# SamsungLabs/nb-asr

Hardware: NVIDIA B200
Metric: train_utterances_per_sec (higher is better)
Workload: dtype bf16

## Files before the change

include/nbasr.h:

```cpp
#ifndef NBASR_H
#define NBASR_H

#include <stdint.h>

#ifdef __cplusplus
extern "C" {
#endif

#define NBASR_F32 0
#define NBASR_BF16 1
#define NBASR_F16 2
#define NBASR_PAD_L 8
#define NBASR_PAD_R 4
#define NBASR_MAX_ADD 3

typedef struct nbasr_epilogue {
  const float* bias;
  int32_t relu20;
  float drop_p;
  uint64_t drop_seed;
  const uint64_t* drop_step;
  int32_t n_add;
  const void* add[NBASR_MAX_ADD];
  int32_t add_dtype;
// ... 49 lines not shown
  const void* w;
  int32_t w_packed;
  nbasr_epilogue epi;
} nbasr_gconv;

int nbasr_gconv_fwd(const nbasr_gconv* p, void* stream);
int nbasr_gconv_chain(const nbasr_gconv* nodes, int n, int fused, void* work, int64_t work_bytes, void* stream);
int64_t nbasr_gconv_chain_work_bytes(int B, int T, int C, int cpg, int n);
int nbasr_pack_gconv_dgrad(const float* w, float* wt, int C, int cpg, int ktaps, void* stream);
int nbasr_pack_gconv_mma(const float* w, void* out, int out_dtype, int C, int cpg, int ktaps, int transposed, void* stream);
int64_t nbasr_gconv_mma_pack_elems(int C, int cpg, int ktaps);
int nbasr_gconv_wgrad(int dtype, const void* dz, const void* x, int B, int T, int Tp, int C, int cpg,
                      int ktaps, int off0, int dstep, float* dw, float* dbias, void* stream);
int nbasr_gconv_wgrad_x(int dz_dtype, const void* dz, const void* x, int x_dtype, float x_scale, int B, int T, int Tp, int C,
                        int cpg, int ktaps, int off0, int dstep, float* dw, float* dbias, void* stream);

int nbasr_eltwise(int src_dtype, const void* src, int64_t ld_src, int B, int T, int Tp, int C,
                  const nbasr_epilogue* epi, void* stream);

int nbasr_colsum(int dtype, const void* x, int B, int T, int Tp, int C, float* out, void* stream);

int nbasr_layernorm_fwd(int dtype, const void* x, void* y, int B, int T, int Tp, int C,
                        const float* gamma, const float* beta, float eps, float* mean, float* rstd,
                        float out_scale, void* y2, void* stream);
int nbasr_layernorm_bwd(int dtype, const void* dy, const void* x, int x_dtype, float x_scale, const float* mean,
                        const float* rstd, const float* gamma, int B, int T, int Tp, int C, void* dx, void* dx2,
                        const uint32_t* mask2, float scale2, int64_t mask_rows, int mask2_w, float* dgamma,
                        float* dbeta, void* stream);

int nbasr_transpose_in(const float* audio, void* out, int dtype, int B, int F, int T, int Tp, float scale, void* stream);
// ... 86 lines not shown
```

nb_asr_b200/_lib.py:

```python
import ctypes as C
import os

from . import _build

F32, BF16, F16 = 0, 1, 2
PAD_L, PAD_R = 8, 4
MAX_ADD = 3

_vp, _i32, _i64, _f32, _u64 = C.c_void_p, C.c_int32, C.c_int64, C.c_float, C.c_uint64


class Epilogue(C.Structure):
    _fields_ = [('bias', _vp), ('relu20', _i32), ('drop_p', _f32), ('drop_seed', _u64), ('drop_step', _vp),
                ('n_add', _i32), ('add', _vp * MAX_ADD), ('add_dtype', _i32), ('out', _vp), ('out_dtype', _i32),
                ('ld_out', _i64), ('mask_out', _vp), ('out2', _vp), ('out2_dtype', _i32), ('mask2', _vp),
                ('scale2', _f32), ('mask_rows', _i64), ('mask_w', _i32), ('mask2_w', _i32), ('accumulate', _i32),
                ('acc_scale', _f32), ('bias_scale', _f32), ('relu_hi', _f32)]


class Gemm(C.Structure):
    _fields_ = [('dtype', _i32), ('a', _vp), ('a_bs', _i64), ('a_rs', _i64), ('nb', _i32), ('nr', _i32),
                ('K', _i32), ('N', _i32), ('w', _vp), ('ldw', _i64), ('o_r0', _i64), ('o_bs', _i64),
                ('o_rs', _i64), ('epi', Epilogue)]


class Wgrad(C.Structure):
    _fields_ = [('dtype', _i32), ('dy', _vp), ('dy_bs', _i64), ('dy_rs', _i64), ('x', _vp), ('x_bs', _i64),
                ('x_rs', _i64), ('nb', _i32), ('nr', _i32), ('M', _i32), ('N', _i32), ('dw', _vp), ('ldw', _i64), ('dbias', _vp)]


class PackJob(C.Structure):
    _fields_ = [('kind', _i32), ('out_dtype', _i32), ('src', _vp), ('dst', _vp), ('n_out', _i64), ('a', _i32 * 8), ('s', _i64 * 3)]


class GConv(C.Structure):
    _fields_ = [('dtype', _i32), ('x', _vp), ('B', _i32), ('T', _i32), ('Tp', _i32), ('C', _i32), ('cpg', _i32),
                ('ktaps', _i32), ('off0', _i32), ('dstep', _i32), ('w', _vp), ('w_packed', _i32), ('epi', Epilogue)]


class GateLayer(C.Structure):
    _fields_ = [('mask', _vp), ('mask_rows', _i64), ('w', _i32), ('C', _i32), ('Tp', _i32), ('T', _i32), ('s', _i32),
                ('reserved', _i32)]


_SIGS = {
    'nbasr_gemm_tn': [C.POINTER(Gemm), _vp],
    'nbasr_gemm_wgrad': [C.POINTER(Wgrad), _vp],
    'nbasr_gconv_fwd': [C.POINTER(GConv), _vp],
    'nbasr_gconv_chain': [C.POINTER(GConv), C.c_int, C.c_int, _vp, _i64, _vp],
    'nbasr_gconv_chain_work_bytes': [C.c_int] * 5,
    'nbasr_pack_gconv_dgrad': [_vp, _vp, C.c_int, C.c_int, C.c_int, _vp],
    'nbasr_pack_gconv_mma': [_vp, _vp, C.c_int, C.c_int, C.c_int, C.c_int, C.c_int, _vp],
    'nbasr_gconv_mma_pack_elems': [C.c_int, C.c_int, C.c_int],
    'nbasr_gconv_wgrad': [C.c_int, _vp, _vp] + [C.c_int] * 8 + [_vp, _vp, _vp],
    'nbasr_gconv_wgrad_x': [C.c_int, _vp, _vp, C.c_int, _f32] + [C.c_int] * 8 + [_vp, _vp, _vp],
    'nbasr_eltwise': [C.c_int, _vp, _i64, C.c_int, C.c_int, C.c_int, C.c_int, C.POINTER(Epilogue), _vp],
    'nbasr_colsum': [C.c_int, _vp, C.c_int, C.c_int, C.c_int, C.c_int, _vp, _vp],
    'nbasr_layernorm_fwd': [C.c_int, _vp, _vp, C.c_int, C.c_int, C.c_int, C.c_int, _vp, _vp, _f32, _vp, _vp, _f32, _vp, _vp],
    'nbasr_layernorm_bwd': [C.c_int, _vp, _vp, C.c_int, _f32, _vp, _vp, _vp, C.c_int, C.c_int, C.c_int, C.c_int, _vp, _vp, _vp,
                            _f32, _i64, C.c_int, _vp, _vp, _vp],
    'nbasr_transpose_in': [_vp, _vp, C.c_int, C.c_int, C.c_int, C.c_int, C.c_int, _f32, _vp],
    'nbasr_transpose_out': [_vp, _vp, C.c_int, C.c_int, C.c_int, C.c_int, _vp],
    'nbasr_param_stats': [_vp, _vp, _vp, _vp, C.c_int, _i64, _vp, _vp, _vp],
    'nbasr_row_gram': [_vp, C.c_int, _i64, _i64, _vp, _vp, _vp, _vp],
    'nbasr_gate_gram': [_vp, C.c_int, _vp, C.c_int, _vp, _vp, _vp],
    'nbasr_gate_gram_work_elems': [C.c_int],
    'nbasr_pack_weight': [_vp, _vp, C.c_int, C.c_int, C.c_int, C.c_int, C.c_int, C.c_int, _i64, _i64, _i64, _vp],
    'nbasr_convert': [_vp, _vp, C.c_int, _i64, _vp],
    'nbasr_lstm_fwd': [_vp, _vp, C.c_int, C.c_int, C.c_int, _vp, C.c_int, _i64, _i64, _i64, _vp, _vp, _vp, _vp, _vp],
    'nbasr_lstm_bwd': [_vp, _i64, _i64, _i64, _vp, _vp, _vp, C.c_int, C.c_int, C.c_int, _vp, _vp, _vp, _vp, _vp],
# ... 60 lines not shown
```

nb_asr_b200/csrc/gconv.cu:

```cuda
#include <algorithm>

#include "common.cuh"
#include "kernels.h"

namespace {

constexpr int G_TT = 64;
constexpr int G_FB = 16;
constexpr int G_MAXHALO = 12;
constexpr int G_NT = 256;

__host__ __device__ inline int slab_channels(int cpg) {
  return cpg == 10 ? 160 : 96;
}
__host__ __device__ inline int wpitch(int cpg, int ktaps) {
  int p = cpg * ktaps;
  return (p & 1) ? p : p + 1;
}

template <typename T>
__global__ void __launch_bounds__(G_NT) gconv_fwd_kernel(nbasr_gconv p) {
  extern __shared__ float smem[];
  const int CS = slab_channels(p.cpg);
  const int halo = (p.ktaps - 1) * p.dstep;
// ... 222 lines not shown
  if (packed) return sm100_gconv_chain(nodes, n, fused, work, work_bytes, as_stream(stream));
  for (int i = 0; i < n; ++i)
    if (nbasr_gconv_fwd(nodes + i, stream)) return 1;
  return 0;
}

int64_t nbasr_gconv_chain_work_bytes(int B, int T, int C, int cpg, int n) { return sm100_gconv_chain_work_bytes(B, T, C, cpg, n); }

int nbasr_pack_gconv_dgrad(const float* w, float* wt, int C, int cpg, int ktaps, void* stream) {
  int total = C * cpg * ktaps;
  pack_gconv_dgrad_kernel<<<(total + 255) / 256, 256, 0, as_stream(stream)>>>(w, wt, C, cpg, ktaps);
  NBASR_CHECK_LAUNCH();
  return 0;
}

int nbasr_gconv_wgrad_x(int dz_dtype, const void* dz, const void* x, int x_dtype, float x_scale, int B, int T, int Tp, int C,
                        int cpg, int ktaps, int off0, int dstep, float* dw, float* dbias, void* stream) {
  NBASR_REQUIRE(cpg == 6 || cpg == 8 || cpg == 10 || cpg == 12, "cpg");
  NBASR_REQUIRE(ktaps <= 7 && (dstep == 1 || dstep == 2), "taps");
  NBASR_REQUIRE(dz_dtype == NBASR_BF16 ? (x_dtype == NBASR_BF16 || x_dtype == NBASR_F16) : (dz_dtype == NBASR_F32 && x_dtype == NBASR_F32),
                "dtypes: bf16 dz with bf16 / fp16 x, or fp32 dz and x");
  if (B <= 0 || T <= 0) return 0;
  if (dz_dtype == NBASR_BF16 && !nbasr_env_flag(NBASR_ENV_FORCE_SIMT))
    return sm100_gconv_wgrad(dz, x, x_dtype == NBASR_F16, x_scale, B, T, Tp, C, cpg, ktaps, off0, dstep, dw, dbias, as_stream(stream));
  if (dbias && nbasr_colsum(dz_dtype, dz, B, T, Tp, C, dbias, stream)) return 1;
  int CS = slab_channels(cpg);
  dim3 grid((C + CS - 1) / CS, B);
  size_t sm = wgrad_smem(cpg);
  auto launch = [&](auto kern, auto dzp, auto xp) {
    static DevOnce attr;
    if (!attr) { cudaFuncSetAttribute(kern, cudaFuncAttributeMaxDynamicSharedMemorySize, 200 * 1024); attr = true; }
    kern<<<grid, G_NT, sm, as_stream(stream)>>>(dzp, xp, x_scale, B, T, Tp, C, cpg, ktaps, off0, dstep, dw);
  };
  if (dz_dtype == NBASR_F32) launch(gconv_wgrad_kernel<float, float>, (const float*)dz, (const float*)x);
  else if (x_dtype == NBASR_F16) launch(gconv_wgrad_kernel<bf16, f16>, (const bf16*)dz, (const f16*)x);
  else launch(gconv_wgrad_kernel<bf16, bf16>, (const bf16*)dz, (const bf16*)x);
  NBASR_CHECK_LAUNCH();
  return 0;
}

int nbasr_gconv_wgrad(int dtype, const void* dz, const void* x, int B, int T, int Tp, int C, int cpg, int ktaps,
                      int off0, int dstep, float* dw, float* dbias, void* stream) {
  return nbasr_gconv_wgrad_x(dtype, dz, x, dtype, 1.f, B, T, Tp, C, cpg, ktaps, off0, dstep, dw, dbias, stream);
}

}
```

nb_asr_b200/csrc/gconv_sm100.cu:

```cuda
#include <cuda.h>

#include "common.cuh"
#include "kernels.h"
#include "sm100_ptx.cuh"
#include "gconv_sm100.cuh"

using namespace sm100;

namespace {

struct GcFwdArgs {
  int B, T, C, OUT, ktaps, dstep, off0;
  int nslabs, ntiles, tiles_per_utt, nlanes, nstage, no_prefetch, w_stable, f16;
  nbasr_epilogue epi;
  int64_t Tp;
};


__global__ void __launch_bounds__(FWD_THREADS, 2)
gconv_mma_fwd_kernel(const __grid_constant__ CUtensorMap tmX, const __grid_constant__ CUtensorMap tmW,
                     const __grid_constant__ CUtensorMap tmO, const __grid_constant__ CUtensorMap tmO2, const GcFwdArgs p) {
  extern __shared__ uint8_t smem_raw[];
  const uint32_t base = (smem_u32(smem_raw) + 1023u) & ~1023u;
  uint8_t* al = smem_raw + (base - smem_u32(smem_raw));
// ... 207 lines not shown
      }
    }
    if (hh == 0 && lane == 0) bulk_wait0();
  }
  tcgen05_fence_before();
  __syncthreads();
  if (warp == W_MMA) {
    tcgen05_fence_after();
    tmem_dealloc(tm, 256);
  }
}

constexpr int DZROWS = 136;
constexpr int DZ_BYTES = DZROWS * 128;
constexpr int WG_STAGE = DZ_BYTES + A_BYTES;
constexpr int WG_SMEM = NSTAGE * WG_STAGE + 1024 + 256;

struct GcWgArgs {
  int B, T, C, cpg, OUT, ktaps, dstep, off0;
  int nslabs, nchunks, nunits, nlanes, dbg;
  int x_f16;
  float x_scale;
  float* dw;
  float* dbias;
};

__global__ void __launch_bounds__(GC_THREADS, 2)
gconv_mma_wgrad_kernel(const __grid_constant__ CUtensorMap tmDZ, const __grid_constant__ CUtensorMap tmX, const GcWgArgs p) {
  extern __shared__ uint8_t smem_raw[];
  const uint32_t base = (smem_u32(smem_raw) + 1023u) & ~1023u;
  uint8_t* al = smem_raw + (base - smem_u32(smem_raw));
  const uint32_t bar0 = base + NSTAGE * WG_STAGE;
  auto full_bar = [&](int s) { return bar0 + 8u * s; };
  auto empty_bar = [&](int s) { return bar0 + 8u * (NSTAGE + s); };
  const uint32_t tfull = bar0 + 8u * (2 * NSTAGE);
  auto ready_bar = [&](int s) { return bar0 + 8u * (2 * NSTAGE + 1 + s); };
  uint32_t* tptr = reinterpret_cast<uint32_t*>(al + NSTAGE * WG_STAGE + 8 * (3 * NSTAGE + 2));
  const int warp = uniform_warp_idx(), lane = threadIdx.x & 31;
  const int slab = blockIdx.x % p.nslabs;
  const int lane_id = blockIdx.x / p.nslabs;
  const int c0 = slab * p.OUT;
  const int cbox = c0 & ~7, coff = c0 - cbox;
  const int npairs = (p.ktaps + 1) / 2;

  if (warp == 4 && lane == 0) {
    prefetch_tmap(&tmDZ);
    prefetch_tmap(&tmX);
    for (int s = 0; s < NSTAGE; ++s) { mbar_init(full_bar(s), 1); mbar_init(empty_bar(s), 1); mbar_init(ready_bar(s), 4); }
    mbar_init(tfull, 1);
    fence_barrier_init();
  }
  if (warp == 5) tmem_alloc(smem_u32(tptr), 256);
  pdl_launch_dependents();
  tcgen05_fence_before();
  __syncthreads();
  tcgen05_fence_after();
  const uint32_t tm = *tptr;
  pdl_wait();
  const bool has_work = lane_id < p.nunits;

  if (warp == 4) {
    if (lane == 0) {
      int stage = 0;
      uint32_t phase = 0;
      for (int u = lane_id; u < p.nunits; u += p.nlanes) {
        const int b = u / p.nchunks, t0 = (u % p.nchunks) * GT;
        mbar_wait(empty_bar(stage), phase ^ 1);
        mbar_expect_tx(full_bar(stage), DZ_BYTES + A_BYTES);
        const uint32_t sa = base + stage * WG_STAGE;
        tma_load_3d(sa, &tmDZ, full_bar(stage), cbox, NBASR_PAD_L + t0 - p.dstep, b);
        tma_load_3d(sa + DZ_BYTES, &tmX, full_bar(stage), cbox, NBASR_PAD_L + t0 + p.off0, b);
        if (++stage == NSTAGE) { stage = 0; phase ^= 1; }
      }
    }
  } else if (warp == 5) {
    if (has_work) {
      const uint32_t idesc = make_idesc(128, 64 * npairs, 1, 1);
      int stage = 0;
      uint32_t phase = 0;
      bool first = true;
      for (int u = lane_id; u < p.nunits; u += p.nlanes) {
        mbar_wait((p.x_f16 || p.dbias) ? ready_bar(stage) : full_bar(stage), phase);
        const uint32_t sa = base + stage * WG_STAGE;
        tcgen05_fence_after();
        const uint64_t ad0 = make_smem_desc(sa, (uint32_t)p.dstep * 128u, 1024);
        const uint64_t bd0 = make_smem_desc(sa + DZ_BYTES, 2u * (uint32_t)p.dstep * 128u, 1024);
        if (elect_one()) {
#pragma unroll
          for (int k = 0; k < GT / 16; ++k)
            if (!(p.dbg & 2048) || k == 0) umma_bf16(tm, ad0 + (uint64_t)(k * 128), bd0 + (uint64_t)(k * 128), idesc, (!first || k > 0) ? 1u : 0u);
          umma_commit(empty_bar(stage));
        }
        __syncwarp();
        first = false;
        if (++stage == NSTAGE) { stage = 0; phase ^= 1; }
      }
      if (elect_one()) umma_commit(tfull);
      __syncwarp();
    }
  } else if (has_work) {
    if (p.x_f16 || p.dbias) {
      constexpr int QROWS = AROWS / 4;
      const int r0 = warp * QROWS;
      int stage = 0;
      uint32_t phase = 0;
      for (int u = lane_id; u < p.nunits; u += p.nlanes) {
        mbar_wait(full_bar(stage), phase);
        uint8_t* xb = al + stage * WG_STAGE + DZ_BYTES;
        if (p.x_f16) {
#pragma unroll 3
          for (int i = lane; i < QROWS * 8; i += 32) {
            const int r = r0 + (i >> 3), ch = i & 7;
            uint4* cp = reinterpret_cast<uint4*>(xb + r * 128 + ch * 16);
            uint4 w = *cp;
            uint32_t* h = &w.x;
#pragma unroll
            for (int e = 0; e < 4; ++e) {
              const float2 f = f16x2_to_f2(h[e]);
              h[e] = f2_to_bf16x2(f.x * p.x_scale, f.y * p.x_scale);
            }
            if (p.dbias && ch == (7 ^ (r & 7))) w.w = (w.w & 0xffffu) | (0x3F80u << 16);
            *cp = w;
          }
        } else {
          for (int r = r0 + lane; r < r0 + QROWS; r += 32)
            *reinterpret_cast<uint16_t*>(xb + r * 128 + ((7 ^ (r & 7)) << 4) + 14) = 0x3F80;
        }
        asm volatile("fence.proxy.async.shared::cta;" ::: "memory");
        __syncwarp();
        if (lane == 0) mbar_arrive(ready_bar(stage));
        if (++stage == NSTAGE) { stage = 0; phase ^= 1; }
      }
    }
    const int q = warp & 3;
    const int m = q * 32 + lane;
    const int half = m >> 6, co_l = m & 63;
    const int co = cbox + co_l;
    const bool row_ok = co_l >= coff && co_l < coff + p.OUT && co < p.C;
    const int g_l = (co_l - coff) / p.cpg;
    const int nco = min(p.OUT, p.C - c0);
    const int nrun = nco * p.cpg * p.ktaps;
    float* g = p.dw + (int64_t)c0 * p.cpg * p.ktaps;
    const int head = min(nrun, (int)(((16u - (uint32_t)(reinterpret_cast<uintptr_t>(g) & 15u)) & 15u) >> 2));
    float* run = reinterpret_cast<float*>(al) + ((4 - head) & 3);
    mbar_wait(tfull, 0);
    tcgen05_fence_after();
    for (int pr = 0; pr < npairs; ++pr) {
      float v[64];
      const uint32_t ta = tm + ((uint32_t)(q * 32) << 16) + pr * 64;
      tmem_ld32(ta, v);
      tmem_ld32(ta + 32, v + 32);
      const int tap = half ? 2 * pr : 2 * pr + 1;
      if (pr == 0 && p.dbias && row_ok && half) atomicAdd(p.dbias + co, v[63]);
      if (row_ok && tap < p.ktaps) {
        float* dst = run + (co_l - coff) * p.cpg * p.ktaps + tap;
#pragma unroll
        for (int i = 0; i < 64; ++i) {
          const int il = i - coff - g_l * p.cpg;
          if (il >= 0 && il < p.cpg) dst[il * p.ktaps] = v[i];
        }
      }
    }
    named_bar_sync(1, 128);
    if (!(p.dbg & 1024)) {
      const int tid = threadIdx.x;
      const int nvec = (nrun - head) >> 2, tail = head + 4 * nvec;
      if (tid < head) atomicAdd(g + tid, run[tid]);
      for (int j = tid; j < nvec; j += 128)
        atomicAdd(reinterpret_cast<float4*>(g + head) + j, reinterpret_cast<const float4*>(run + head)[j]);
      if (tail + tid < nrun) atomicAdd(g + tail + tid, run[tail + tid]);
    }
  }
  tcgen05_fence_before();
  __syncthreads();
  if (warp == 5) {
    tcgen05_fence_after();
    tmem_dealloc(tm, 256);
  }
}

template <typename T>
__global__ void pack_gconv_mma_kernel(const float* __restrict__ w, T* __restrict__ out, int C, int cpg, int ktaps, int OUT,
                                      int nslabs, int transposed) {
  int64_t idx = (int64_t)blockIdx.x * blockDim.x + threadIdx.x;
  int64_t total = (int64_t)nslabs * ktaps * NW * 64;
  if (idx >= total) return;
  int kk = (int)(idx % 64);
  int n = (int)((idx / 64) % NW);
  int j = (int)((idx / (64 * NW)) % ktaps);
  int s = (int)(idx / ((int64_t)64 * NW * ktaps));
  int c0 = s * OUT;
  int cn = c0 + n, ck = c0 + kk;
// ... 41 lines not shown
  if (sm100_get_map(o1, 3, dx, sx, bo, &tmO, 0)) return 1;
  if (sm100_get_map(o2, 3, dx, sx, bo, &tmO2, 0)) return 1;
  NBASR_REQUIRE(!g->epi.mask_out || g->epi.mask_w == a.OUT, "grouped-conv mask planes are slab wide");
  size_t smem = (size_t)a.ktaps * WTAP_BYTES + (size_t)a.nstage * A_BYTES + 2 * OSTAGE_BYTES + 1024 + 256 + 1024;
  static DevOnce attr;
  if (!attr) {
    cudaError_t e = cudaFuncSetAttribute(gconv_mma_fwd_kernel, cudaFuncAttributeMaxDynamicSharedMemorySize, FWD_SMEM_BUDGET);
    if (e != cudaSuccess) return nbasr_fail("gconv_mma_fwd smem attr: %s", cudaGetErrorString(e));
    attr = true;
  }
  cudaError_t le = launch_pdl(gconv_mma_fwd_kernel, dim3(a.nslabs * a.nlanes), dim3(FWD_THREADS), smem, st, 1, tmX, tmW, tmO, tmO2, a);
  if (le != cudaSuccess) return nbasr_fail("gconv_mma_fwd launch: %s", cudaGetErrorString(le));
  return 0;
}

int sm100_gconv_wgrad(const void* dz, const void* x, int x_f16, float x_scale, int B, int T, int Tp, int C, int cpg, int ktaps,
                      int off0, int dstep, float* dw, float* dbias, cudaStream_t st) {
  GcWgArgs a{};
  a.x_f16 = x_f16;
  a.x_scale = x_scale;
  a.B = B; a.T = T; a.C = C; a.cpg = cpg; a.OUT = wg_slab_out(cpg); a.ktaps = ktaps; a.dstep = dstep; a.off0 = off0;
  NBASR_REQUIRE(off0 >= -NBASR_PAD_L && (ktaps - 1) * dstep <= AROWS - GT && dstep <= DZROWS - GT, "tap reach");
  a.nslabs = (C + a.OUT - 1) / a.OUT;
  a.nchunks = (T + dstep + GT - 1) / GT;
  a.nunits = a.nchunks * B;
  int slots = GCONV_SLOTS * nbasr_sm_count();
  a.nlanes = std::max(1, std::min(a.nunits, slots / a.nslabs));
  a.dw = dw;
  a.dbias = dbias;
  a.dbg = nbasr_env_chain_dbg();
  CUtensorMap tmDZ, tmX;
  uint64_t dd[3] = {(uint64_t)C, (uint64_t)Tp, (uint64_t)B};
  int64_t sd[3] = {1, C, (int64_t)Tp * C};
  uint32_t bz[3] = {64, DZROWS, 1};
  uint32_t bx[3] = {64, AROWS, 1};
  if (sm100_get_map(dz, 3, dd, sd, bz, &tmDZ)) return 1;
  if (sm100_get_map(x, 3, dd, sd, bx, &tmX)) return 1;
  static DevOnce attr;
  if (!attr) {
    cudaError_t e = cudaFuncSetAttribute(gconv_mma_wgrad_kernel, cudaFuncAttributeMaxDynamicSharedMemorySize, WG_SMEM);
    if (e != cudaSuccess) return nbasr_fail("gconv_mma_wgrad smem attr: %s", cudaGetErrorString(e));
    attr = true;
  }
  cudaError_t le = launch_pdl(gconv_mma_wgrad_kernel, dim3(a.nslabs * a.nlanes), dim3(GC_THREADS), (size_t)WG_SMEM, st, 1, tmDZ, tmX, a);
  if (le != cudaSuccess) return nbasr_fail("gconv_mma_wgrad launch: %s", cudaGetErrorString(le));
  return 0;
}

extern "C" int nbasr_pack_gconv_mma(const float* w, void* out, int out_dtype, int C, int cpg, int ktaps, int transposed, void* stream) {
  int OUT = slab_out(cpg);
  int nslabs = (C + OUT - 1) / OUT;
  int64_t total = (int64_t)nslabs * ktaps * NW * 64;
  NBASR_REQUIRE(out_dtype == NBASR_BF16 || out_dtype == NBASR_F16, "16-bit pack");
  const unsigned grid = (unsigned)((total + 255) / 256);
  if (out_dtype == NBASR_F16) pack_gconv_mma_kernel<f16><<<grid, 256, 0, as_stream(stream)>>>(w, (f16*)out, C, cpg, ktaps, OUT, nslabs, transposed);
  else pack_gconv_mma_kernel<bf16><<<grid, 256, 0, as_stream(stream)>>>(w, (bf16*)out, C, cpg, ktaps, OUT, nslabs, transposed);
  NBASR_CHECK_LAUNCH();
  return 0;
}
// ... 6 lines not shown
```

nb_asr_b200/csrc/gconv_sm100.cuh:

```cuda
#pragma once
#include "sm100_ptx.cuh"

namespace {
using namespace sm100;

constexpr int GT = 128;
constexpr int AROWS = 144;
constexpr int A_BYTES = AROWS * 128;
constexpr int NW = 48;
constexpr int WTAP_BYTES = NW * 128;
constexpr int NSTAGE = 3;
constexpr int NACC = 4;
constexpr int GC_THREADS = 192;
constexpr int FWD_THREADS = 448;
constexpr int NEPI = 384;
constexpr int OSTAGE_BYTES = GT * NW * 2;
constexpr int FWD_SMEM_BUDGET = 112 * 1024;

__host__ __device__ inline int slab_out(int cpg) { return cpg == 10 ? 40 : 48; }
__host__ __device__ inline int wg_slab_out(int cpg) { return (56 / cpg) * cpg; }
__host__ __device__ inline int fwd_nstage(int ktaps) {
  int n = (FWD_SMEM_BUDGET - 3072 - ktaps * WTAP_BYTES - 2 * OSTAGE_BYTES) / A_BYTES;
  return n > 4 ? 4 : n;
}


constexpr int GCONV_SLOTS = 2;
}
// ... 1 lines not shown
```

nb_asr_b200/csrc/kernels.h:

```cpp
#pragma once
#include <cuda_runtime.h>
#include <stdint.h>

#include "../../include/nbasr.h"

enum NbasrEnvFlag { NBASR_ENV_FORCE_SIMT = 0, NBASR_ENV_NO_PDL, NBASR_ENV_GCONV_NO_PREFETCH, NBASR_ENV_LSTM_SS, NBASR_ENV_DEBUG,
                    NBASR_ENV_GEMM_DIRECT_EPI, NBASR_ENV_WGRAD_V1, NBASR_ENV_COUNT };
bool nbasr_env_flag(int which);
int nbasr_env_gemm_bn();
int nbasr_env_gemm_l2pf();
int nbasr_env_chain_dbg();
double nbasr_env_wgrad_epi_us();

struct DevOnce {
  unsigned long long mask = 0;
  static int dev() { int d = 0; cudaGetDevice(&d); return d & 63; }
  bool operator!() const { return !((mask >> dev()) & 1ull); }
  DevOnce& operator=(bool v) { if (v) mask |= 1ull << dev(); return *this; }
};

#ifdef __CUDACC__
#include <utility>
template <typename... KArgs, typename... Args>
inline cudaError_t launch_pdl(void (*kern)(KArgs...), dim3 grid, dim3 block, size_t smem, cudaStream_t st, int cluster_x,
// ... 29 lines not shown
  int64_t o_r0, o_bs, o_rs;
  nbasr_epilogue epi;
};
int simt_gemm_launch(const SimtGemmArgs& a, cudaStream_t st);

int sm100_gemm_tn_pair(const nbasr_gemm* p, cudaStream_t st);
int sm100_gemm_wgrad_pair(const nbasr_wgrad* p, cudaStream_t st);

struct CUtensorMap_st;
int sm100_get_map(const void* base, int rank, const uint64_t* dims, const int64_t* strides_el, const uint32_t* box,
                  CUtensorMap_st* out, int swizzle128 = 1);

int sm100_gconv_fwd(const nbasr_gconv* p, cudaStream_t st);
int sm100_gconv_chain(const nbasr_gconv* nodes, int n, int fused, void* work, int64_t work_bytes, cudaStream_t st);
int64_t sm100_gconv_chain_work_bytes(int B, int T, int C, int cpg, int n);
int sm100_gconv_wgrad(const void* dz, const void* x, int x_f16, float x_scale, int B, int T, int Tp, int C, int cpg, int ktaps,
                      int off0, int dstep, float* dw, float* dbias, cudaStream_t st);

int sm100_lstm_fwd(const float* gx, const void* w_packed, int T, int B, int H, void* h_seq, int h_dtype, int64_t h_bs, int64_t h_rs,
                   float* gates, float* cstate, cudaStream_t st);
int sm100_lstm_bwd(const float* dh_seq, int64_t dh_bs, int64_t dh_rs, const void* w_packed, const float* gates, const float* cstate,
                   int T, int B, int H, float* dgx, void* dgx_bf16, cudaStream_t st);

int ln2_fwd(const void* x, void* y, int f16, int B, int T, int Tp, int C, const float* gamma, const float* beta, float eps, float* mean,
            float* rstd, float out_scale, void* y2, cudaStream_t st);
int ln2_bwd(const void* dy, const void* x, int x_f16, float x_scale, const float* mean, const float* rstd, const float* gamma, int B, int T,
            int Tp, int C, void* dx, void* dx2, const uint32_t* mask2, float scale2, int64_t mask_rows, int mask2_w, float* dgamma,
            float* dbeta, cudaStream_t st);
```

nb_asr_b200/engine.py:

```python
import collections
import ctypes as C
import functools
import math
import os

import torch

from . import _lib
from ._lib import BF16, F16, F32, PAD_L, PAD_R, Epilogue, GConv, Gemm, Wgrad
from .model import CELLS_PER_BLOCK, CONV_EDGES, FEATURES, FILTERS, HIDDEN, TR_STRIDES, PadConvRelu, pad_rule

HP = 512
ACT_SCALE = 32.0


def _ptr(t, off_elems=0):
    return t.data_ptr() + off_elems * t.element_size()


def dense_wgrad_inputs(arch, use_norm, use_rnn, input_dropout=False):
    ops = [nd[0] for nd in arch]
    names = {'input'}
    for i, ncells in enumerate(CELLS_PER_BLOCK):
        cin = f'b{i}.ln'
# ... 734 lines not shown
                         last['mask'].w if dz_t is not None else 32,
                         self.G(crec['name'] + '.norm_layer.weight'), self.G(crec['name'] + '.norm_layer.bias'))
                    pool.append(gout)
                else:
                    g[nn_] = gout
                    if last['op'] != 'zero':
                        dz_t = dz[nn_ - 1]
                        dzb[nn_ - 1] = dz_t
                        epi = self._epi(Cc, out2=dz_t.data_ptr(), mask2=last['mask'], scale2=dscale, mask_rows=geo.rows)
                        call(bwd, lib.nbasr_eltwise, dt, gout.data_ptr(), Cc, B, Ti, Tp, Cc, C.byref(epi))
                        pl.keep.append(epi)
                chain, chain_wg = [], []

                def flush_bwd():
                    flush_chain(bwd, chain)
                    for a_ in chain_wg:
                        call(bwd, lib.nbasr_gconv_wgrad_x, *a_)
                    del chain_wg[:]

                for j in range(nn_ - 1, -1, -1):
                    nrec = nodes[j]
                    op, pn = nrec['op'], nrec['pn']
                    src = outs[j]
                    adds = [g[k + 1].data_ptr() for k in range(j, nn_) if nodes[k]['branches'][j]]
                    g[j] = pool.pop()
                    o2, m2 = 0, None
                    if j >= 1 and nodes[j - 1]['op'] != 'zero':
                        dzb[j - 1] = dz[j - 1]
                        o2, m2 = dzb[j - 1].data_ptr(), nodes[j - 1]['mask']
                    epi = self._epi(Cc, adds=adds, out=g[j].data_ptr() if (need_g(j) or not o2) else 0, out2=o2, mask2=m2, scale2=dscale,
                                    mask_rows=geo.rows)
                    if op not in CONV_EDGES:
                        flush_bwd()
                    if op == 'zero':
                        call(bwd, lib.nbasr_eltwise, dt, None, Cc, B, Ti, Tp, Cc, C.byref(epi))
                        pl.keep.append(epi)
                    elif op == 'linear':
                        d = dzb[j]
                        fuse = dt == BF16
                        wgrad(bwd, _ptr(d, PAD_L * Cc), Tp * Cc, Cc, _ptr(Bc(src), PAD_L * Cc), Tp * Cc, Cc, B, Ti, Cc, Cc,
                              self.G(pn + '.linear.weight'), Cc, dbias=self.G(pn + '.linear.bias') if fuse else None)
                        if not fuse:
                            call(bwd, lib.nbasr_colsum, dt, d.data_ptr(), B, Ti, Tp, Cc, self.G(pn + '.linear.bias'))
                        gemm(bwd, _ptr(d, PAD_L * Cc), Tp * Cc, Cc, B, Ti, Cc, Cc, self.wt[pn].data_ptr(), Cc, PAD_L, Tp, 1, epi)
                    else:
                        d = dzb[j]
                        k, dd, lp = nrec['k'], nrec['d'], nrec['lp']
                        chain_wg.append((dt, d.data_ptr(), src.data_ptr(), adt, 1.0 / S, B, Ti, Tp, Cc, Cc // 100, k, -lp, dd,
                                         self.G(pn + '.conv.weight'), self.G(pn + '.conv.bias')))
                        gc = GConv()
                        gc.dtype, gc.x, gc.B, gc.T, gc.Tp, gc.C, gc.cpg = dt, d.data_ptr(), B, Ti, Tp, Cc, Cc // 100
                        gc.ktaps, gc.off0, gc.dstep, gc.w = k, lp - (k - 1) * dd, dd, self.wt[pn].data_ptr()
                        gc.w_packed = 3 if dt == BF16 else 0
                        gc.epi = epi
                        chain.append(gc)
                        pl.keep.append(gc)
                flush_bwd()
                for k in range(1, nn_ + 1):
                    pool.append(g[k])
                gout = g[0]
            dzc = dz[0]
            if i == 0:
                dz_blk0 = dzc
            lname, cname = self.block_ln[i], self.block_conv[i]
# ... 160 lines not shown
```

nb_asr_b200/profiling.py:

```python
import collections
import ctypes as C

import torch

from . import _lib
from ._lib import BF16, GConv, Gemm, Wgrad


def _struct_of(arg, typ):
    obj = getattr(arg, '_obj', None)
    return obj if isinstance(obj, typ) else None


def op_work(fn_name, args, es):
    if fn_name == 'nbasr_gemm_tn':
        g = _struct_of(args[0], Gemm)
        rows = g.nb * g.nr
        flops = 2.0 * rows * g.K * g.N
        a_cols = min(g.K, g.a_rs) if g.a_rs > 0 else g.K
        n_o = g.epi.n_add + (1 if g.epi.out else 0) + (1 if (g.epi.out2 and g.epi.mask2) else 0)
        byts = rows * a_cols * es + g.N * g.K * es + rows * g.N * es * n_o
        return f'gemm_tn K={g.K} N={g.N}', flops, byts
    if fn_name == 'nbasr_gemm_wgrad':
        w = _struct_of(args[0], Wgrad)
# ... 7 lines not shown
        el = g.B * g.T * g.C
        n_t = 1 + g.epi.n_add + (1 if g.epi.out else 0) + (1 if (g.epi.out2 and g.epi.mask2) else 0)
        n_m = (1 if g.epi.mask_out else 0) + (1 if g.epi.mask2 else 0)
        return f'gconv C={g.C} k={g.ktaps} d={g.dstep}', 2.0 * el * g.cpg * g.ktaps, el * es * n_t + el * n_m / 8.0
    if fn_name == 'nbasr_gconv_chain':
        fl = by = 0.0
        for i in range(args[1]):
            _, f1, b1 = op_work('nbasr_gconv_fwd', (C.byref(args[0][i]),), es)
            fl, by = fl + f1, by + b1
        g = args[0][0]
        return f'gconv C={g.C} chain of {args[1]}', fl, by
    if fn_name in ('nbasr_gconv_wgrad', 'nbasr_gconv_wgrad_x'):
        B, T, Tp, Cc, cpg, k = args[3:9] if fn_name == 'nbasr_gconv_wgrad' else args[5:11]
        el = B * T * Cc
        return f'gconv_wgrad C={Cc} k={k}', 2.0 * el * cpg * k, el * es * 2
    if fn_name in ('nbasr_layernorm_fwd', 'nbasr_layernorm_bwd'):
        if fn_name.endswith('fwd'):
            B, T, Tp, Cc = args[3:7]
            return f'ln_fwd C={Cc}', 0.0, B * T * Cc * es * 2
        B, T, Tp, Cc = args[8:12]
        n_out = (1 if args[12] else 0) + (1 if args[13] else 0)
        return f'ln_bwd C={Cc}', 0.0, B * T * Cc * es * (2 + n_out)
    if fn_name == 'nbasr_eltwise':
        B, T, Tp, Cc = args[3:7]
        return f'eltwise C={Cc}', 0.0, B * T * Cc * es * 2
    if fn_name == 'nbasr_colsum':
        B, T, Tp, Cc = args[2:6]
        return f'colsum C={Cc}', 0.0, B * T * Cc * (2 if args[0] == BF16 else 4)
    return fn_name.replace('nbasr_', ''), 0.0, 0.0

# ... 50 lines not shown
```

Before: 8811.

## Batch grouped-conv weight-gradient problems into one persistent kernel with double-buffered TMEM

Adds a multi-problem gconv wgrad entry point so up to four per-layer weight-gradient computations in a backward chain run in a single launch. The kernel gains separate epilogue warps and a double-buffered TMEM accumulator, so reduction of one problem can overlap MMA of the next. Stage count rises from 3 to 5, the block grows to 320 threads, and occupancy drops to one block per SM. The aim is to remove per-layer launch overhead and pipeline bubbles, at the risk of lower parallelism since lanes are now capped by SM count instead of twice the slots.

```diff
diff --git a/include/nbasr.h b/include/nbasr.h
--- a/include/nbasr.h
+++ b/include/nbasr.h
@@ -87,6 +87,16 @@
                       int ktaps, int off0, int dstep, float* dw, float* dbias, void* stream);
 int nbasr_gconv_wgrad_x(int dz_dtype, const void* dz, const void* x, int x_dtype, float x_scale, int B, int T, int Tp, int C,
                         int cpg, int ktaps, int off0, int dstep, float* dw, float* dbias, void* stream);
+#define NBASR_GCONV_WGRAD_MAXP 4
+typedef struct nbasr_gconv_wgrad_problem {
+  const void* dz;
+  const void* x;
+  float* dw;
+  float* dbias;
+  int32_t ktaps, off0, dstep, reserved;
+} nbasr_gconv_wgrad_problem;
+int nbasr_gconv_wgrad_multi(int n, const nbasr_gconv_wgrad_problem* problems, int dz_dtype, int x_dtype, float x_scale, int B,
+                            int T, int Tp, int C, int cpg, void* stream);
 
 int nbasr_eltwise(int src_dtype, const void* src, int64_t ld_src, int B, int T, int Tp, int C,
                   const nbasr_epilogue* epi, void* stream);
diff --git a/nb_asr_b200/_lib.py b/nb_asr_b200/_lib.py
--- a/nb_asr_b200/_lib.py
+++ b/nb_asr_b200/_lib.py
@@ -38,6 +38,14 @@
                 ('ktaps', _i32), ('off0', _i32), ('dstep', _i32), ('w', _vp), ('w_packed', _i32), ('epi', Epilogue)]
 
 
+class GconvWgradProblem(C.Structure):
+    _fields_ = [('dz', _vp), ('x', _vp), ('dw', _vp), ('dbias', _vp), ('ktaps', _i32), ('off0', _i32), ('dstep', _i32),
+                ('reserved', _i32)]
+
+
+GCONV_WGRAD_MAXP = 4
+
+
 class GateLayer(C.Structure):
     _fields_ = [('mask', _vp), ('mask_rows', _i64), ('w', _i32), ('C', _i32), ('Tp', _i32), ('T', _i32), ('s', _i32),
                 ('reserved', _i32)]
@@ -54,6 +62,7 @@
     'nbasr_gconv_mma_pack_elems': [C.c_int, C.c_int, C.c_int],
     'nbasr_gconv_wgrad': [C.c_int, _vp, _vp] + [C.c_int] * 8 + [_vp, _vp, _vp],
     'nbasr_gconv_wgrad_x': [C.c_int, _vp, _vp, C.c_int, _f32] + [C.c_int] * 8 + [_vp, _vp, _vp],
+    'nbasr_gconv_wgrad_multi': [C.c_int, C.POINTER(GconvWgradProblem), C.c_int, C.c_int, _f32] + [C.c_int] * 5 + [_vp],
     'nbasr_eltwise': [C.c_int, _vp, _i64, C.c_int, C.c_int, C.c_int, C.c_int, C.POINTER(Epilogue), _vp],
     'nbasr_colsum': [C.c_int, _vp, C.c_int, C.c_int, C.c_int, C.c_int, _vp, _vp],
     'nbasr_layernorm_fwd': [C.c_int, _vp, _vp, C.c_int, C.c_int, C.c_int, C.c_int, _vp, _vp, _f32, _vp, _vp, _f32, _vp, _vp],
diff --git a/nb_asr_b200/csrc/gconv.cu b/nb_asr_b200/csrc/gconv.cu
--- a/nb_asr_b200/csrc/gconv.cu
+++ b/nb_asr_b200/csrc/gconv.cu
@@ -260,15 +260,8 @@
   return 0;
 }
 
-int nbasr_gconv_wgrad_x(int dz_dtype, const void* dz, const void* x, int x_dtype, float x_scale, int B, int T, int Tp, int C,
-                        int cpg, int ktaps, int off0, int dstep, float* dw, float* dbias, void* stream) {
-  NBASR_REQUIRE(cpg == 6 || cpg == 8 || cpg == 10 || cpg == 12, "cpg");
-  NBASR_REQUIRE(ktaps <= 7 && (dstep == 1 || dstep == 2), "taps");
-  NBASR_REQUIRE(dz_dtype == NBASR_BF16 ? (x_dtype == NBASR_BF16 || x_dtype == NBASR_F16) : (dz_dtype == NBASR_F32 && x_dtype == NBASR_F32),
-                "dtypes: bf16 dz with bf16 / fp16 x, or fp32 dz and x");
-  if (B <= 0 || T <= 0) return 0;
-  if (dz_dtype == NBASR_BF16 && !nbasr_env_flag(NBASR_ENV_FORCE_SIMT))
-    return sm100_gconv_wgrad(dz, x, x_dtype == NBASR_F16, x_scale, B, T, Tp, C, cpg, ktaps, off0, dstep, dw, dbias, as_stream(stream));
+static int simt_gconv_wgrad(int dz_dtype, const void* dz, const void* x, int x_dtype, float x_scale, int B, int T, int Tp, int C,
+                            int cpg, int ktaps, int off0, int dstep, float* dw, float* dbias, void* stream) {
   if (dbias && nbasr_colsum(dz_dtype, dz, B, T, Tp, C, dbias, stream)) return 1;
   int CS = slab_channels(cpg);
   dim3 grid((C + CS - 1) / CS, B);
@@ -285,6 +278,29 @@
   return 0;
 }
 
+int nbasr_gconv_wgrad_multi(int n, const nbasr_gconv_wgrad_problem* pb, int dz_dtype, int x_dtype, float x_scale, int B, int T,
+                            int Tp, int C, int cpg, void* stream) {
+  NBASR_REQUIRE(n >= 1 && n <= NBASR_GCONV_WGRAD_MAXP, "1 .. NBASR_GCONV_WGRAD_MAXP problems");
+  NBASR_REQUIRE(cpg == 6 || cpg == 8 || cpg == 10 || cpg == 12, "cpg");
+  for (int i = 0; i < n; ++i) NBASR_REQUIRE(pb[i].ktaps <= 7 && (pb[i].dstep == 1 || pb[i].dstep == 2), "taps");
+  NBASR_REQUIRE(dz_dtype == NBASR_BF16 ? (x_dtype == NBASR_BF16 || x_dtype == NBASR_F16) : (dz_dtype == NBASR_F32 && x_dtype == NBASR_F32),
+                "dtypes: bf16 dz with bf16 / fp16 x, or fp32 dz and x");
+  if (B <= 0 || T <= 0) return 0;
+  if (dz_dtype == NBASR_BF16 && !nbasr_env_flag(NBASR_ENV_FORCE_SIMT))
+    return sm100_gconv_wgrad(n, pb, x_dtype == NBASR_F16, x_scale, B, T, Tp, C, cpg, as_stream(stream));
+  for (int i = 0; i < n; ++i)
+    if (simt_gconv_wgrad(dz_dtype, pb[i].dz, pb[i].x, x_dtype, x_scale, B, T, Tp, C, cpg, pb[i].ktaps, pb[i].off0, pb[i].dstep,
+                         pb[i].dw, pb[i].dbias, stream))
+      return 1;
+  return 0;
+}
+
+int nbasr_gconv_wgrad_x(int dz_dtype, const void* dz, const void* x, int x_dtype, float x_scale, int B, int T, int Tp, int C,
+                        int cpg, int ktaps, int off0, int dstep, float* dw, float* dbias, void* stream) {
+  nbasr_gconv_wgrad_problem pb{dz, x, dw, dbias, ktaps, off0, dstep, 0};
+  return nbasr_gconv_wgrad_multi(1, &pb, dz_dtype, x_dtype, x_scale, B, T, Tp, C, cpg, stream);
+}
+
 int nbasr_gconv_wgrad(int dtype, const void* dz, const void* x, int B, int T, int Tp, int C, int cpg, int ktaps,
                       int off0, int dstep, float* dw, float* dbias, void* stream) {
   return nbasr_gconv_wgrad_x(dtype, dz, x, dtype, 1.f, B, T, Tp, C, cpg, ktaps, off0, dstep, dw, dbias, stream);
diff --git a/nb_asr_b200/csrc/gconv_sm100.cu b/nb_asr_b200/csrc/gconv_sm100.cu
--- a/nb_asr_b200/csrc/gconv_sm100.cu
+++ b/nb_asr_b200/csrc/gconv_sm100.cu
@@ -245,103 +245,121 @@
 constexpr int DZROWS = 136;
 constexpr int DZ_BYTES = DZROWS * 128;
 constexpr int WG_STAGE = DZ_BYTES + A_BYTES;
-constexpr int WG_SMEM = NSTAGE * WG_STAGE + 1024 + 256;
-
-struct GcWgArgs {
-  int B, T, C, cpg, OUT, ktaps, dstep, off0;
-  int nslabs, nchunks, nunits, nlanes, dbg;
-  int x_f16;
-  float x_scale;
+constexpr int WG_RUN_BYTES = 16384;
+constexpr int WG_SMEM = NSTAGE * WG_STAGE + WG_RUN_BYTES + 256 + 1024;
+constexpr int WG_ACC_COLS = 256;
+
+constexpr int WG_MAXP = NBASR_GCONV_WGRAD_MAXP;
+
+struct GcWgProb {
+  int ktaps, dstep, off0, nchunks, nunits;
   float* dw;
   float* dbias;
 };
 
-__global__ void __launch_bounds__(GC_THREADS, 2)
-gconv_mma_wgrad_kernel(const __grid_constant__ CUtensorMap tmDZ, const __grid_constant__ CUtensorMap tmX, const GcWgArgs p) {
+struct GcWgArgs {
+  int B, T, C, cpg, OUT, nslabs, nlanes, nprob, dbg;
+  int x_f16;
+  float x_scale;
+  GcWgProb pr[WG_MAXP];
+};
+
+struct GcWgMaps {
+  CUtensorMap dz[WG_MAXP], x[WG_MAXP];
+};
+
+__global__ void __launch_bounds__(GC_THREADS, 1)
+gconv_mma_wgrad_kernel(const __grid_constant__ GcWgMaps maps, const __grid_constant__ GcWgArgs p) {
   extern __shared__ uint8_t smem_raw[];
   const uint32_t base = (smem_u32(smem_raw) + 1023u) & ~1023u;
   uint8_t* al = smem_raw + (base - smem_u32(smem_raw));
-  const uint32_t bar0 = base + NSTAGE * WG_STAGE;
+  const uint32_t bar0 = base + NSTAGE * WG_STAGE + WG_RUN_BYTES;
   auto full_bar = [&](int s) { return bar0 + 8u * s; };
   auto empty_bar = [&](int s) { return bar0 + 8u * (NSTAGE + s); };
-  const uint32_t tfull = bar0 + 8u * (2 * NSTAGE);
-  auto ready_bar = [&](int s) { return bar0 + 8u * (2 * NSTAGE + 1 + s); };
-  uint32_t* tptr = reinterpret_cast<uint32_t*>(al + NSTAGE * WG_STAGE + 8 * (3 * NSTAGE + 2));
+  auto ready_bar = [&](int s) { return bar0 + 8u * (2 * NSTAGE + s); };
+  auto tfull_bar = [&](int a) { return bar0 + 8u * (3 * NSTAGE + a); };
+  auto tempty_bar = [&](int a) { return bar0 + 8u * (3 * NSTAGE + 2 + a); };
+  uint32_t* tptr = reinterpret_cast<uint32_t*>(al + NSTAGE * WG_STAGE + WG_RUN_BYTES + 8 * (3 * NSTAGE + 4));
+  float* runbuf = reinterpret_cast<float*>(al + NSTAGE * WG_STAGE);
+  constexpr int W_PROD = 8, W_MMA = 9;
   const int warp = uniform_warp_idx(), lane = threadIdx.x & 31;
   const int slab = blockIdx.x % p.nslabs;
   const int lane_id = blockIdx.x / p.nslabs;
   const int c0 = slab * p.OUT;
   const int cbox = c0 & ~7, coff = c0 - cbox;
-  const int npairs = (p.ktaps + 1) / 2;
-
-  if (warp == 4 && lane == 0) {
-    prefetch_tmap(&tmDZ);
-    prefetch_tmap(&tmX);
+
+  if (warp == W_PROD && lane == 0) {
+    for (int i = 0; i < p.nprob; ++i) { prefetch_tmap(&maps.dz[i]); prefetch_tmap(&maps.x[i]); }
     for (int s = 0; s < NSTAGE; ++s) { mbar_init(full_bar(s), 1); mbar_init(empty_bar(s), 1); mbar_init(ready_bar(s), 4); }
-    mbar_init(tfull, 1);
+    for (int a = 0; a < 2; ++a) { mbar_init(tfull_bar(a), 1); mbar_init(tempty_bar(a), 4); }
     fence_barrier_init();
   }
-  if (warp == 5) tmem_alloc(smem_u32(tptr), 256);
+  if (warp == W_MMA) tmem_alloc(smem_u32(tptr), 2 * WG_ACC_COLS);
   pdl_launch_dependents();
   tcgen05_fence_before();
   __syncthreads();
   tcgen05_fence_after();
   const uint32_t tm = *tptr;
   pdl_wait();
-  const bool has_work = lane_id < p.nunits;
-
-  if (warp == 4) {
+
+  if (warp == W_PROD) {
     if (lane == 0) {
       int stage = 0;
       uint32_t phase = 0;
-      for (int u = lane_id; u < p.nunits; u += p.nlanes) {
-        const int b = u / p.nchunks, t0 = (u % p.nchunks) * GT;
-        mbar_wait(empty_bar(stage), phase ^ 1);
-        mbar_expect_tx(full_bar(stage), DZ_BYTES + A_BYTES);
-        const uint32_t sa = base + stage * WG_STAGE;
-        tma_load_3d(sa, &tmDZ, full_bar(stage), cbox, NBASR_PAD_L + t0 - p.dstep, b);
-        tma_load_3d(sa + DZ_BYTES, &tmX, full_bar(stage), cbox, NBASR_PAD_L + t0 + p.off0, b);
-        if (++stage == NSTAGE) { stage = 0; phase ^= 1; }
-      }
-    }
-  } else if (warp == 5) {
-    if (has_work) {
-      const uint32_t idesc = make_idesc(128, 64 * npairs, 1, 1);
-      int stage = 0;
-      uint32_t phase = 0;
-      bool first = true;
-      for (int u = lane_id; u < p.nunits; u += p.nlanes) {
-        mbar_wait((p.x_f16 || p.dbias) ? ready_bar(stage) : full_bar(stage), phase);
+      for (int pi = 0; pi < p.nprob; ++pi) {
+        const GcWgProb& pr = p.pr[pi];
+        for (int u = lane_id; u < pr.nunits; u += p.nlanes) {
+          const int b = u / pr.nchunks, t0 = (u % pr.nchunks) * GT;
+          mbar_wait(empty_bar(stage), phase ^ 1);
+          mbar_expect_tx(full_bar(stage), DZ_BYTES + A_BYTES);
+          const uint32_t sa = base + stage * WG_STAGE;
+          tma_load_3d(sa, &maps.dz[pi], full_bar(stage), cbox, NBASR_PAD_L + t0 - pr.dstep, b);
+          tma_load_3d(sa + DZ_BYTES, &maps.x[pi], full_bar(stage), cbox, NBASR_PAD_L + t0 + pr.off0, b);
+          if (++stage == NSTAGE) { stage = 0; phase ^= 1; }
+        }
+      }
+    }
+  } else if (warp == W_MMA) {
+    int stage = 0;
+    uint32_t phase = 0;
+    for (int j = 0; j < p.nprob; ++j) {
+      const GcWgProb& pr = p.pr[j];
+      const int acc = j & 1;
+      const uint32_t idesc = make_idesc(128, 64 * ((pr.ktaps + 1) / 2), 1, 1);
+      mbar_wait(tempty_bar(acc), ((j >> 1) & 1) ^ 1);
+      for (int u = lane_id; u < pr.nunits; u += p.nlanes) {
+        mbar_wait(ready_bar(stage), phase);
         const uint32_t sa = base + stage * WG_STAGE;
         tcgen05_fence_after();
-        const uint64_t ad0 = make_smem_desc(sa, (uint32_t)p.dstep * 128u, 1024);
-        const uint64_t bd0 = make_smem_desc(sa + DZ_BYTES, 2u * (uint32_t)p.dstep * 128u, 1024);
+        const uint64_t ad0 = make_smem_desc(sa, (uint32_t)pr.dstep * 128u, 1024);
+        const uint64_t bd0 = make_smem_desc(sa + DZ_BYTES, 2u * (uint32_t)pr.dstep * 128u, 1024);
         if (elect_one()) {
 #pragma unroll
           for (int k = 0; k < GT / 16; ++k)
-            if (!(p.dbg & 2048) || k == 0) umma_bf16(tm, ad0 + (uint64_t)(k * 128), bd0 + (uint64_t)(k * 128), idesc, (!first || k > 0) ? 1u : 0u);
+            if (!(p.dbg & 2048) || k == 0)
+              umma_bf16(tm + acc * WG_ACC_COLS, ad0 + (uint64_t)(k * 128), bd0 + (uint64_t)(k * 128), idesc, (u > lane_id || k > 0) ? 1u : 0u);
           umma_commit(empty_bar(stage));
         }
         __syncwarp();
-        first = false;
         if (++stage == NSTAGE) { stage = 0; phase ^= 1; }
       }
-      if (elect_one()) umma_commit(tfull);
+      if (elect_one()) umma_commit(tfull_bar(acc));
       __syncwarp();
     }
-  } else if (has_work) {
-    if (p.x_f16 || p.dbias) {
-      constexpr int QROWS = AROWS / 4;
-      const int r0 = warp * QROWS;
-      int stage = 0;
-      uint32_t phase = 0;
-      for (int u = lane_id; u < p.nunits; u += p.nlanes) {
+  } else if (warp >= 4) {
+    constexpr int QROWS = AROWS / 4;
+    const int r0 = (warp - 4) * QROWS;
+    int stage = 0;
+    uint32_t phase = 0;
+    for (int pi = 0; pi < p.nprob; ++pi) {
+      const bool ones = p.pr[pi].dbias != nullptr;
+      for (int u = lane_id; u < p.pr[pi].nunits; u += p.nlanes) {
         mbar_wait(full_bar(stage), phase);
         uint8_t* xb = al + stage * WG_STAGE + DZ_BYTES;
         if (p.x_f16) {
 #pragma unroll 3
-          for (int i = lane; i < QROWS * 8; i += 32) {
-            const int r = r0 + (i >> 3), ch = i & 7;
+          for (int c = lane; c < QROWS * 8; c += 32) {
+            const int r = r0 + (c >> 3), ch = c & 7;
             uint4* cp = reinterpret_cast<uint4*>(xb + r * 128 + ch * 16);
             uint4 w = *cp;
             uint32_t* h = &w.x;
@@ -350,10 +368,10 @@
               const float2 f = f16x2_to_f2(h[e]);
               h[e] = f2_to_bf16x2(f.x * p.x_scale, f.y * p.x_scale);
             }
-            if (p.dbias && ch == (7 ^ (r & 7))) w.w = (w.w & 0xffffu) | (0x3F80u << 16);
+            if (ones && ch == (7 ^ (r & 7))) w.w = (w.w & 0xffffu) | (0x3F80u << 16);
             *cp = w;
           }
-        } else {
+        } else if (ones) {
           for (int r = r0 + lane; r < r0 + QROWS; r += 32)
             *reinterpret_cast<uint16_t*>(xb + r * 128 + ((7 ^ (r & 7)) << 4) + 14) = 0x3F80;
         }
@@ -363,50 +381,59 @@
         if (++stage == NSTAGE) { stage = 0; phase ^= 1; }
       }
     }
-    const int q = warp & 3;
-    const int m = q * 32 + lane;
+  } else {
+    const int m = warp * 32 + lane;
     const int half = m >> 6, co_l = m & 63;
+    const int tid = threadIdx.x;
     const int co = cbox + co_l;
     const bool row_ok = co_l >= coff && co_l < coff + p.OUT && co < p.C;
     const int g_l = (co_l - coff) / p.cpg;
     const int nco = min(p.OUT, p.C - c0);
-    const int nrun = nco * p.cpg * p.ktaps;
-    float* g = p.dw + (int64_t)c0 * p.cpg * p.ktaps;
-    const int head = min(nrun, (int)(((16u - (uint32_t)(reinterpret_cast<uintptr_t>(g) & 15u)) & 15u) >> 2));
-    float* run = reinterpret_cast<float*>(al) + ((4 - head) & 3);
-    mbar_wait(tfull, 0);
-    tcgen05_fence_after();
-    for (int pr = 0; pr < npairs; ++pr) {
-      float v[64];
-      const uint32_t ta = tm + ((uint32_t)(q * 32) << 16) + pr * 64;
-      tmem_ld32(ta, v);
-      tmem_ld32(ta + 32, v + 32);
-      const int tap = half ? 2 * pr : 2 * pr + 1;
-      if (pr == 0 && p.dbias && row_ok && half) atomicAdd(p.dbias + co, v[63]);
-      if (row_ok && tap < p.ktaps) {
-        float* dst = run + (co_l - coff) * p.cpg * p.ktaps + tap;
-#pragma unroll
-        for (int i = 0; i < 64; ++i) {
-          const int il = i - coff - g_l * p.cpg;
-          if (il >= 0 && il < p.cpg) dst[il * p.ktaps] = v[i];
-        }
-      }
-    }
-    named_bar_sync(1, 128);
-    if (!(p.dbg & 1024)) {
-      const int tid = threadIdx.x;
-      const int nvec = (nrun - head) >> 2, tail = head + 4 * nvec;
-      if (tid < head) atomicAdd(g + tid, run[tid]);
-      for (int j = tid; j < nvec; j += 128)
-        atomicAdd(reinterpret_cast<float4*>(g + head) + j, reinterpret_cast<const float4*>(run + head)[j]);
-      if (tail + tid < nrun) atomicAdd(g + tail + tid, run[tail + tid]);
+    for (int j = 0; j < p.nprob; ++j) {
+      const GcWgProb& pr = p.pr[j];
+      const int acc = j & 1;
+      const int kt = pr.ktaps;
+      const int nrun = nco * p.cpg * kt;
+      float* g = pr.dw + (int64_t)c0 * p.cpg * kt;
+      const int head = min(nrun, (int)(((16u - (uint32_t)(reinterpret_cast<uintptr_t>(g) & 15u)) & 15u) >> 2));
+      float* run = runbuf + ((4 - head) & 3);
+      named_bar_sync(1, 128);
+      mbar_wait(tfull_bar(acc), (j >> 1) & 1);
+      tcgen05_fence_after();
+      for (int q = 0; q < (kt + 1) / 2; ++q) {
+        float v[64];
+        const uint32_t ta = tm + ((uint32_t)(warp * 32) << 16) + acc * WG_ACC_COLS + q * 64;
+        tmem_ld32(ta, v);
+        tmem_ld32(ta + 32, v + 32);
+        const int tap = half ? 2 * q : 2 * q + 1;
+        if (q == 0 && pr.dbias && row_ok && half) atomicAdd(pr.dbias + co, v[63]);
+        if (row_ok && tap < kt) {
+          float* dst = run + (co_l - coff) * p.cpg * kt + tap;
+#pragma unroll
+          for (int e = 0; e < 64; ++e) {
+            const int il = e - coff - g_l * p.cpg;
+            if (il >= 0 && il < p.cpg) dst[il * kt] = v[e];
+          }
+        }
+      }
+      tcgen05_fence_before();
+      __syncwarp();
+      if (lane == 0) mbar_arrive(tempty_bar(acc));
+      named_bar_sync(1, 128);
+      if (!(p.dbg & 1024)) {
+        const int nvec = (nrun - head) >> 2, tail = head + 4 * nvec;
+        if (tid < head) atomicAdd(g + tid, run[tid]);
+        for (int e = tid; e < nvec; e += 128)
+          atomicAdd(reinterpret_cast<float4*>(g + head) + e, reinterpret_cast<const float4*>(run + head)[e]);
+        if (tail + tid < nrun) atomicAdd(g + tail + tid, run[tail + tid]);
+      }
     }
   }
   tcgen05_fence_before();
   __syncthreads();
-  if (warp == 5) {
+  if (warp == W_MMA) {
     tcgen05_fence_after();
-    tmem_dealloc(tm, 256);
+    tmem_dealloc(tm, 2 * WG_ACC_COLS);
   }
 }
 
@@ -478,35 +505,43 @@
   return 0;
 }
 
-int sm100_gconv_wgrad(const void* dz, const void* x, int x_f16, float x_scale, int B, int T, int Tp, int C, int cpg, int ktaps,
-                      int off0, int dstep, float* dw, float* dbias, cudaStream_t st) {
+int sm100_gconv_wgrad(int n, const nbasr_gconv_wgrad_problem* pb, int x_f16, float x_scale, int B, int T, int Tp, int C,
+                      int cpg, cudaStream_t st) {
+  NBASR_REQUIRE(n >= 1 && n <= WG_MAXP, "1 .. NBASR_GCONV_WGRAD_MAXP problems");
   GcWgArgs a{};
+  GcWgMaps maps;
   a.x_f16 = x_f16;
   a.x_scale = x_scale;
-  a.B = B; a.T = T; a.C = C; a.cpg = cpg; a.OUT = wg_slab_out(cpg); a.ktaps = ktaps; a.dstep = dstep; a.off0 = off0;
-  NBASR_REQUIRE(off0 >= -NBASR_PAD_L && (ktaps - 1) * dstep <= AROWS - GT && dstep <= DZROWS - GT, "tap reach");
+  a.B = B; a.T = T; a.C = C; a.cpg = cpg; a.OUT = wg_slab_out(cpg); a.nprob = n;
   a.nslabs = (C + a.OUT - 1) / a.OUT;
-  a.nchunks = (T + dstep + GT - 1) / GT;
-  a.nunits = a.nchunks * B;
-  int slots = GCONV_SLOTS * nbasr_sm_count();
-  a.nlanes = std::max(1, std::min(a.nunits, slots / a.nslabs));
-  a.dw = dw;
-  a.dbias = dbias;
   a.dbg = nbasr_env_chain_dbg();
-  CUtensorMap tmDZ, tmX;
   uint64_t dd[3] = {(uint64_t)C, (uint64_t)Tp, (uint64_t)B};
   int64_t sd[3] = {1, C, (int64_t)Tp * C};
   uint32_t bz[3] = {64, DZROWS, 1};
   uint32_t bx[3] = {64, AROWS, 1};
-  if (sm100_get_map(dz, 3, dd, sd, bz, &tmDZ)) return 1;
-  if (sm100_get_map(x, 3, dd, sd, bx, &tmX)) return 1;
+  int min_units = 1 << 30;
+  for (int i = 0; i < n; ++i) {
+    const nbasr_gconv_wgrad_problem& q = pb[i];
+    NBASR_REQUIRE(q.off0 >= -NBASR_PAD_L && (q.ktaps - 1) * q.dstep <= AROWS - GT && q.dstep <= DZROWS - GT, "tap reach");
+    GcWgProb& r = a.pr[i];
+    r.ktaps = q.ktaps; r.dstep = q.dstep; r.off0 = q.off0;
+    r.nchunks = (T + q.dstep + GT - 1) / GT;
+    r.nunits = r.nchunks * B;
+    r.dw = q.dw;
+    r.dbias = q.dbias;
+    min_units = std::min(min_units, r.nunits);
+    if (sm100_get_map(q.dz, 3, dd, sd, bz, &maps.dz[i])) return 1;
+    if (sm100_get_map(q.x, 3, dd, sd, bx, &maps.x[i])) return 1;
+  }
+  for (int i = n; i < WG_MAXP; ++i) { maps.dz[i] = maps.dz[0]; maps.x[i] = maps.x[0]; }
+  a.nlanes = std::max(1, std::min(min_units, nbasr_sm_count() / a.nslabs));
   static DevOnce attr;
   if (!attr) {
     cudaError_t e = cudaFuncSetAttribute(gconv_mma_wgrad_kernel, cudaFuncAttributeMaxDynamicSharedMemorySize, WG_SMEM);
     if (e != cudaSuccess) return nbasr_fail("gconv_mma_wgrad smem attr: %s", cudaGetErrorString(e));
     attr = true;
   }
-  cudaError_t le = launch_pdl(gconv_mma_wgrad_kernel, dim3(a.nslabs * a.nlanes), dim3(GC_THREADS), (size_t)WG_SMEM, st, 1, tmDZ, tmX, a);
+  cudaError_t le = launch_pdl(gconv_mma_wgrad_kernel, dim3(a.nslabs * a.nlanes), dim3(GC_THREADS), (size_t)WG_SMEM, st, 1, maps, a);
   if (le != cudaSuccess) return nbasr_fail("gconv_mma_wgrad launch: %s", cudaGetErrorString(le));
   return 0;
 }
diff --git a/nb_asr_b200/csrc/gconv_sm100.cuh b/nb_asr_b200/csrc/gconv_sm100.cuh
--- a/nb_asr_b200/csrc/gconv_sm100.cuh
+++ b/nb_asr_b200/csrc/gconv_sm100.cuh
@@ -9,9 +9,9 @@
 constexpr int A_BYTES = AROWS * 128;
 constexpr int NW = 48;
 constexpr int WTAP_BYTES = NW * 128;
-constexpr int NSTAGE = 3;
+constexpr int NSTAGE = 5;
 constexpr int NACC = 4;
-constexpr int GC_THREADS = 192;
+constexpr int GC_THREADS = 320;
 constexpr int FWD_THREADS = 448;
 constexpr int NEPI = 384;
 constexpr int OSTAGE_BYTES = GT * NW * 2;
diff --git a/nb_asr_b200/csrc/kernels.h b/nb_asr_b200/csrc/kernels.h
--- a/nb_asr_b200/csrc/kernels.h
+++ b/nb_asr_b200/csrc/kernels.h
@@ -67,8 +67,8 @@
 int sm100_gconv_fwd(const nbasr_gconv* p, cudaStream_t st);
 int sm100_gconv_chain(const nbasr_gconv* nodes, int n, int fused, void* work, int64_t work_bytes, cudaStream_t st);
 int64_t sm100_gconv_chain_work_bytes(int B, int T, int C, int cpg, int n);
-int sm100_gconv_wgrad(const void* dz, const void* x, int x_f16, float x_scale, int B, int T, int Tp, int C, int cpg, int ktaps,
-                      int off0, int dstep, float* dw, float* dbias, cudaStream_t st);
+int sm100_gconv_wgrad(int n, const nbasr_gconv_wgrad_problem* pb, int x_f16, float x_scale, int B, int T, int Tp, int C,
+                      int cpg, cudaStream_t st);
 
 int sm100_lstm_fwd(const float* gx, const void* w_packed, int T, int B, int H, void* h_seq, int h_dtype, int64_t h_bs, int64_t h_rs,
                    float* gates, float* cstate, cudaStream_t st);
diff --git a/nb_asr_b200/engine.py b/nb_asr_b200/engine.py
--- a/nb_asr_b200/engine.py
+++ b/nb_asr_b200/engine.py
@@ -7,7 +7,7 @@
 import torch
 
 from . import _lib
-from ._lib import BF16, F16, F32, PAD_L, PAD_R, Epilogue, GConv, Gemm, Wgrad
+from ._lib import BF16, F16, F32, GCONV_WGRAD_MAXP, PAD_L, PAD_R, Epilogue, GConv, GconvWgradProblem, Gemm, Wgrad
 from .model import CELLS_PER_BLOCK, CONV_EDGES, FEATURES, FILTERS, HIDDEN, TR_STRIDES, PadConvRelu, pad_rule
 
 HP = 512
@@ -772,8 +772,10 @@
 
                 def flush_bwd():
                     flush_chain(bwd, chain)
-                    for a_ in chain_wg:
-                        call(bwd, lib.nbasr_gconv_wgrad_x, *a_)
+                    for i0 in range(0, len(chain_wg), GCONV_WGRAD_MAXP):
+                        grp = chain_wg[i0:i0 + GCONV_WGRAD_MAXP]
+                        probs = (GconvWgradProblem * len(grp))(*grp)
+                        call(bwd, lib.nbasr_gconv_wgrad_multi, len(grp), probs, dt, adt, 1.0 / S, B, Ti, Tp, Cc, Cc // 100)
                     del chain_wg[:]
 
                 for j in range(nn_ - 1, -1, -1):
@@ -804,8 +806,8 @@
                     else:
                         d = dzb[j]
                         k, dd, lp = nrec['k'], nrec['d'], nrec['lp']
-                        chain_wg.append((dt, d.data_ptr(), src.data_ptr(), adt, 1.0 / S, B, Ti, Tp, Cc, Cc // 100, k, -lp, dd,
-                                         self.G(pn + '.conv.weight'), self.G(pn + '.conv.bias')))
+                        chain_wg.append(GconvWgradProblem(d.data_ptr(), src.data_ptr(), self.G(pn + '.conv.weight'),
+                                                          self.G(pn + '.conv.bias'), k, -lp, dd))
                         gc = GConv()
                         gc.dtype, gc.x, gc.B, gc.T, gc.Tp, gc.C, gc.cpg = dt, d.data_ptr(), B, Ti, Tp, Cc, Cc // 100
                         gc.ktaps, gc.off0, gc.dstep, gc.w = k, lp - (k - 1) * dd, dd, self.wt[pn].data_ptr()
diff --git a/nb_asr_b200/profiling.py b/nb_asr_b200/profiling.py
--- a/nb_asr_b200/profiling.py
+++ b/nb_asr_b200/profiling.py
@@ -45,6 +45,12 @@
         B, T, Tp, Cc, cpg, k = args[3:9] if fn_name == 'nbasr_gconv_wgrad' else args[5:11]
         el = B * T * Cc
         return f'gconv_wgrad C={Cc} k={k}', 2.0 * el * cpg * k, el * es * 2
+    if fn_name == 'nbasr_gconv_wgrad_multi':
+        n, probs = args[0], args[1]
+        B, T, Tp, Cc, cpg = args[5:10]
+        el = B * T * Cc
+        ks = [probs[i].ktaps for i in range(n)]
+        return f'gconv_wgrad C={Cc} k={"+".join(map(str, ks))}', 2.0 * el * cpg * sum(ks), el * es * 2 * n
     if fn_name in ('nbasr_layernorm_fwd', 'nbasr_layernorm_bwd'):
         if fn_name.endswith('fwd'):
             B, T, Tp, Cc = args[3:7]
```

New measurement: 9047, median of 6. 1.03x the previous value.
